# ishine/minimax-speech

Hardware: AMD Instinct MI355X
Metric: 24 kHz audio-seconds generated per wall-second per node (CosyVoice2-0.5B-shaped LM + flow + DAC-VAE, end to end) (higher is better)
Workload: dtype bf16

## Files before the change

### include/mmx_hip.h

```cpp
#ifndef MMX_HIP_H
#define MMX_HIP_H
#include <stdint.h>
#ifdef __cplusplus
extern "C" {
#endif

#ifndef __HIP__
typedef struct ihipStream_t* hipStream_t;
#endif

#define MMX_F32 0
#define MMX_BF16 1
#define MMX_X2 2
#define MMX_X3 3
#define MMX_X2W 0x12
#define MMX_X3W 0x13
#define MMX_H2 4
#define MMX_H2W 0x14

#define MMX_ACT_NONE 0
#define MMX_ACT_LRELU 1
#define MMX_ACT_GELU 2
#define MMX_ACT_SILU 3
#define MMX_ACT_MISH 4
// ... 70 lines not shown
int mmx_attn_flash_x(const float* q, int64_t ldq, int64_t q_bs, const float* k, int64_t ldk, int64_t k_bs,
                     const float* v, int64_t ldv, int64_t v_bs, float* out, int64_t ldo, int64_t o_bs,
                     int B, int H, int T, float scale, const float* keymask, int64_t km_bs, int chunk,
                     int q_begin, const int32_t* klen, hipStream_t stream);
int mmx_attn_flash_xs(const void* qk, int64_t ldqk, int64_t qk_bs, const void* vt, int64_t ldvt, int64_t vt_bs,
                      float* out, int64_t ldo, int64_t o_bs, int B, int H, int T, float scale, const float* keymask,
                      int64_t km_bs, int chunk, int q_begin, const int32_t* klen, int form, hipStream_t stream);
int mmx_attn_relpos_bf16(const void* q, int64_t ldq, int64_t q_bs, const void* k, int64_t ldk, int64_t k_bs,
                         const void* vt, int64_t ldvt, int64_t vt_bs, const void* pos, int64_t ldp,
                         const float* pos_u, const float* pos_v, void* out, int64_t ldo, int64_t o_bs,
                         int B, int H, int T, float scale, int chunk, const int32_t* klen, hipStream_t stream);

int mmx_attn_flash_fp8(const void* q, int64_t ldq, int64_t q_bs, const void* k, int64_t ldk, int64_t k_bs,
                       const void* vt, int64_t ldvt, int64_t vt_bs, void* out, int64_t ldo, int64_t o_bs,
                       int B, int H, int T, float scale, const float* keymask, int64_t km_bs, int chunk, int q_begin,
                       const int32_t* klen, hipStream_t stream);

int mmx_conv_cin1(const float* x, int64_t x_bs, int T, int C, int k, const float* w, const float* bias, float slope,
                  const float* alpha, float* out_f32, void* out_act, int batch, int dtype, hipStream_t stream);
int mmx_vae_sample(const float* ml, const float* noise, int64_t rows, int D, float* z, float* m, float* logs,
                   hipStream_t stream);
int mmx_mask_rows(void* x, int64_t rows, int C, const float* rowmask, int dtype, hipStream_t stream);
int mmx_pool_rows(const float* x, int64_t x_bs, int rows, int C, int batch, const float* mask, int64_t m_bs, void* out,
                  int64_t ldo, int dtype, hipStream_t stream);
int mmx_prefetch4(const void* p0, int64_t n0, const void* p1, int64_t n1, const void* p2, int64_t n2, const void* p3, int64_t n3,
                  void* sink, int workgroups, hipStream_t stream);
int mmx_resample_linear(const float* x, int64_t rows, int T, int T2, float* out, hipStream_t stream);

int mmx_conv_cout1_tanh(const void* act, int64_t a_bs, int T, int C, int k, const float* w, const float* bias,
                        float slope, int use_tanh, float* out, int64_t o_bs, int batch, int dtype, hipStream_t stream);

#define MMX_X_PACKED 1
#define MMX_OUT_PACKED 2
int mmx_pack_skinny(const void* w, int64_t ldw, int N, int K, const float* kscale, int interleave_half,
                    void* wp, int dtype, hipStream_t stream);
int mmx_skinny_gemm(const void* x, int x_dtype, int64_t ldx, int B, int K, int N, const void* wp,
                    const float* bias, int rs, float eps, int epi, float* out_f32, int64_t ldo_f,
                    void* out_act, int64_t ldo_a, int dtype, int flags, const float* kgamma, hipStream_t stream);

int mmx_decode_prep(const float* x, int64_t ldx, int B, int K, const float* gamma, float* h, int64_t ldh, void* xs,
                    float* ssq, int dtype, hipStream_t stream);
int mmx_skinny2(const void* xs, int B, int K, int N, const void* wp, const float* bias, const float* ssq_in, float eps,
                int epi, float* out, int64_t ldo, void* xs_out, const float* gamma_next, float* ssq_out,
                int tiles_per_wg, int ksplit, float* part, int64_t part_floats, int32_t* tickets, int dtype,
                hipStream_t stream);

int mmx_rope_kv_store(const float* qkv, int64_t ldqkv, int64_t qkv_bs, int B, int rows, int Hq, int Hkv, int D,
                      const float* inv_freq, const int32_t* pos, void* q_out, int64_t ldq, int64_t q_bs,
                      void* kc, void* vc, const int32_t* block_table, int max_pages, int page,
                      int dtype, hipStream_t stream);
int mmx_paged_attn(const void* q, int64_t ldq, int64_t q_bs, int B, int rows, int Hq, int Hkv, int D, float scale,
                   const int32_t* pos, const void* kc, const void* vc, const int32_t* block_table, int max_pages,
                   int page, void* out, int64_t ldo, int64_t o_bs, int dtype, hipStream_t stream);
#define MMX_DA_PACKED 1
#define MMX_DA_PER_HEAD 2
#define MMX_DA_SPLIT 4
#define MMX_DA_H2 8
#define MMX_DA_ONE_HEAD 16
int mmx_decode_attn(const float* qkv, int64_t ldqkv, int B, int Hq, int Hkv, int D, const float* inv_freq,
                    const float* rope_tab, const int32_t* pos, void* kc, void* vc, const int32_t* block_table, int max_pages, int page,
                    float scale, void* out, int64_t ldo, int dtype, int out_packed, hipStream_t stream);
int mmx_decode_attn_fin(const float* qkv, int64_t ldqkv, int B, int Hq, int Hkv, int D, const float* inv_freq,
                        const float* rope_tab, const int32_t* pos, const int32_t* finished, void* kc, void* vc,
                        const int32_t* block_table, int max_pages, int page, float scale, void* out, int64_t ldo, int dtype,
                        int out_packed, hipStream_t stream);
int mmx_swiglu(const float* gu, int64_t ldgu, int rows, int I, void* out, int64_t ldo, int dtype, hipStream_t stream);

int mmx_sample_step(const float* logits, int64_t ldl, int V, int B, int eos_id, int top_k, float top_p,
                    int win_size, float tau_r, uint64_t seed, int32_t* state, int32_t* out_tokens, int max_out,
                    int32_t* sampled, const int32_t* forced, const float* speech_emb, int E, float* next_x,
                    int64_t ldx, float* logp_out, hipStream_t stream);
int mmx_sample_step_tab(const float* logits, int64_t ldl, int V, int B, int eos_id, const int32_t* samp, int32_t* state,
                        int32_t* out_tokens, int max_out, int32_t* sampled, const int32_t* forced, const float* speech_emb,
                        int E, float* next_x, int64_t ldx, float* logp_out, hipStream_t stream);

typedef struct MmxEstNext {
    const void* wqkv;
    const float* n1g;
    const float* n1b;
    void* q_out;
    void* vt_out;
    int64_t q_bs, vt_bs;
    int32_t ldq, ldvt;
} MmxEstNext;
typedef struct MmxEstTailParams {
    const void* ao;
    float* x;
    const void* wo;
    const void* w1;
    const void* w2;
    const float* bo;
    const float* b1;
    const float* b2;
    const float* n3g;
    const float* n3b;
    const float* rowmask;
    void* act_out;
    int64_t ao_bs, x_bs, rm_bs, act_bs;
    int32_t ldao, act_ld, B, T;
    int32_t t_begin;
    float eps;
    MmxEstNext next;
} MmxEstTailParams;
typedef struct MmxEstResnetParams {
    const void* a_in;
    float* x;
// ... 88 lines not shown
```

### minimax-speech_amd/csrc/elementwise.hip

```cpp
#include "common.h"
#include <type_traits>

template <int V> using ic = std::integral_constant<int, V>;

template <typename T, int MAXV, int ACT>
__global__ __launch_bounds__(256) void rownorm_kernel(
    const float* __restrict__ x, long ldx, long x_bs, int rows, int C,
    const float* __restrict__ gamma, const float* __restrict__ beta, float eps, int rms, int act,
    const float* __restrict__ rowmask, long rm_bs, const float* __restrict__ addvec, long av_bs,
    float* __restrict__ outf, long ldo_f, long of_bs, T* __restrict__ outa, long ldo_a, long oa_bs) {
    constexpr bool PRECISE = sizeof(T) == 4;
    const int lane = threadIdx.x & 63, wave = threadIdx.x >> 6;
    const int b = blockIdx.y;
    const int row = blockIdx.x * 4 + wave;
    if (row >= rows) return;
    const float* xr = x + (long)b * x_bs + (long)row * ldx;
    float v[MAXV];
    float s = 0.f;
#pragma unroll
    for (int i = 0; i < MAXV; ++i) {
        int c = lane + i * 64;
        v[i] = c < C ? xr[c] : 0.f;
        s += v[i];
    }
// ... 128 lines not shown
                            void* h, int64_t ldh, int dtype, hipStream_t stream) {
    dtype = MMX_ACT_DTYPE(dtype);
    MMX_CHECK_ARG(x && h && B > 0 && T_ > 0 && C > 0 && ldh >= 4 * C && x_mod > 0);
    dim3 grid(T_, B);
    return dispatch_dtype(dtype, [&](auto el) {
        hipLaunchKernelGGL(est_pack_kernel<decltype(el)>, grid, dim3(128), 0, stream, x, x_bs, x_mod, mu, spks, cond, T_, C, (decltype(el)*)h, ldh);
        return launch_status();
    });
}

template <typename T>
__global__ void sinusoidal_kernel(const float* __restrict__ t, int dim, float scale, T* __restrict__ out) {
    const int b = blockIdx.x;
    const int half = dim / 2;
    const float k = logf(10000.f) / (float)(half - 1);
    for (int i = threadIdx.x; i < dim; i += blockDim.x) {
        int j = i < half ? i : i - half;
        float e = scale * t[b] * expf((float)j * -k);
        out[(long)b * dim + i] = Cvt<T>::from_f(i < half ? sinf(e) : cosf(e));
    }
}
extern "C" int mmx_sinusoidal_emb(const float* t, int B, int dim, float scale, void* out, int dtype, hipStream_t stream) {
    dtype = MMX_ACT_DTYPE(dtype);
    MMX_CHECK_ARG(t && out && B > 0 && dim >= 4 && dim % 2 == 0);
    return dispatch_dtype(dtype, [&](auto el) {
        hipLaunchKernelGGL(sinusoidal_kernel<decltype(el)>, dim3(B), dim3(128), 0, stream, t, dim, scale, (decltype(el)*)out);
        return launch_status();
    });
}

__global__ void cfg_euler_kernel(float* __restrict__ x, const float* __restrict__ dc, const float* __restrict__ du,
                                 float cfg, float dt, long n) {
    long i = (long)blockIdx.x * blockDim.x + threadIdx.x;
    if (i < n) x[i] = x[i] + dt * ((1.0f + cfg) * dc[i] - cfg * du[i]);
}
extern "C" int mmx_cfg_euler(float* x, const float* d_cond, const float* d_uncond, float cfg, float dt, int64_t n,
                             hipStream_t stream) {
    MMX_CHECK_ARG(x && d_cond && d_uncond && n > 0);
    hipLaunchKernelGGL(cfg_euler_kernel, dim3((unsigned)((n + 255) / 256)), dim3(256), 0, stream, x, d_cond, d_uncond, cfg, dt, (long)n);
    MMX_LAUNCH_CHECK();
    return MMX_OK;
}

template <typename T>
__global__ __launch_bounds__(256) void conv_cout1_kernel(const T* __restrict__ act, long a_bs, int Tn, int C, int k,
                                                         const float* __restrict__ w, const float* __restrict__ bias,
                                                         float slope, int use_tanh, float* __restrict__ out, long o_bs) {
    extern __shared__ __attribute__((aligned(16))) char smem[];
    float* ws = reinterpret_cast<float*>(smem);
    T* xs = reinterpret_cast<T*>(ws + k * C);
    const int b = blockIdx.y;
    const int t0 = blockIdx.x * 256;
    const int pad = (k - 1) / 2;
    const T* a = act + (long)b * a_bs;
    for (int i = threadIdx.x; i < k * C; i += 256) ws[i] = w[i];
    const int nrow = 256 + k - 1;
    for (int i = threadIdx.x; i < nrow * C; i += 256) {
        int r = i / C, c = i % C;
        long t = (long)t0 + r - pad;
        xs[i] = (t >= 0 && t < Tn) ? a[t * C + c] : Cvt<T>::from_f(0.f);
    }
    __syncthreads();
    const int t = t0 + threadIdx.x;
    if (t >= Tn) return;
    float acc = bias ? bias[0] : 0.f;
    const T* xr = xs + threadIdx.x * C;
    for (int i = 0; i < k * C; ++i) acc += Cvt<T>::to_f(xr[i]) * ws[i];
    acc = acc > 0.f ? acc : acc * slope;
    out[(long)b * o_bs + t] = use_tanh ? tanhf(acc) : fminf(fmaxf(acc, -1.f), 1.f);
}
extern "C" int mmx_conv_cout1_tanh(const void* act, int64_t a_bs, int T_, int C, int k, const float* w, const float* bias,
                                   float slope, int use_tanh, float* out, int64_t o_bs, int batch, int dtype, hipStream_t stream) {
    dtype = MMX_ACT_DTYPE(dtype);
    MMX_CHECK_ARG(act && w && out && T_ > 0 && C > 0 && k > 0 && (k & 1) && batch > 0);
    dim3 grid((T_ + 255) / 256, batch);
    size_t esz = dtype == MMX_BF16 ? 2 : 4;
    size_t lds = (size_t)k * C * 4 + (size_t)(256 + k - 1) * C * esz;
    MMX_CHECK_ARG(lds <= 160 * 1024);
    return dispatch_dtype(dtype, [&](auto el) {
        MMX_LDS_OPT_IN(conv_cout1_kernel<decltype(el)>, lds);
        hipLaunchKernelGGL(conv_cout1_kernel<decltype(el)>, grid, dim3(256), lds, stream, (const decltype(el)*)act, a_bs, T_, C, k, w, bias, slope, use_tanh, out, o_bs);
        return launch_status();
    });
}

template <typename T>
__global__ __launch_bounds__(256) void conv_cin1_kernel(const float* __restrict__ x, long x_bs, int Tn, int C, int k,
                                                        const float* __restrict__ w, const float* __restrict__ bias, float slope,
                                                        const float* __restrict__ alpha, float* __restrict__ outf, T* __restrict__ outa) {
    constexpr bool PRECISE = sizeof(T) == 4;
    extern __shared__ __attribute__((aligned(16))) char smem[];
    float* xs = reinterpret_cast<float*>(smem);
    float* ws = xs + (256 + k - 1);
    const int b = blockIdx.y, t0 = blockIdx.x * 256, pad = (k - 1) / 2;
    const float* xb = x + (long)b * x_bs;
    for (int i = threadIdx.x; i < 256 + k - 1; i += 256) {
        long t = (long)t0 + i - pad;
        xs[i] = (t >= 0 && t < Tn) ? xb[t] : 0.f;
    }
    for (int i = threadIdx.x; i < C * k; i += 256) ws[i] = w[i];
    __syncthreads();
    const int cg = C / 8;
    for (int item = threadIdx.x; item < 256 * cg; item += 256) {
        const int ts = item / cg, c0 = (item % cg) * 8;
        const int t = t0 + ts;
        if (t >= Tn) continue;
        float v[8];
#pragma unroll
        for (int e = 0; e < 8; ++e) {
            float a = bias ? bias[c0 + e] : 0.f;
            for (int j = 0; j < k; ++j) a += ws[(c0 + e) * k + j] * xs[ts + j];
            a = a > 0.f ? a : a * slope;
            v[e] = a;
        }
        const long o = ((long)b * Tn + t) * C + c0;
        if (outf) {
#pragma unroll
            for (int e = 0; e < 8; ++e) outf[o + e] = v[e];
        }
        if (outa) {
#pragma unroll
            for (int e = 0; e < 8; ++e) outa[o + e] = Cvt<T>::from_f(alpha ? snake_apply<PRECISE>(v[e], alpha[c0 + e]) : v[e]);
        }
    }
}
extern "C" int mmx_conv_cin1(const float* x, int64_t x_bs, int T_, int C, int k, const float* w, const float* bias, float slope,
                             const float* alpha, float* out_f32, void* out_act, int batch, int dtype, hipStream_t stream) {
    dtype = MMX_ACT_DTYPE(dtype);
    MMX_CHECK_ARG(x && w && (out_f32 || out_act) && T_ > 0 && C > 0 && C % 8 == 0 && k > 0 && (k & 1) && batch > 0);
    dim3 grid((T_ + 255) / 256, batch);
// ... 221 lines not shown
```

### minimax-speech_amd/csrc/llm.hip

```cpp
#include "act_layout.h"
#include <type_traits>

template <typename T>
__global__ void pack_skinny_kernel(const T* __restrict__ w, long ldw, int N, int K, const float* __restrict__ kscale,
                                   int half, T* __restrict__ wp) {
    constexpr int E = sizeof(T) == 2 ? 8 : 4;
    constexpr int KB = E * 4;
    const long total = (long)((N + 15) / 16) * (K / KB) * 64 * E;
    for (long idx = (long)blockIdx.x * blockDim.x + threadIdx.x; idx < total; idx += (long)gridDim.x * blockDim.x) {
        int j = idx % E;
        long t = idx / E;
        int lane = t % 64;
        t /= 64;
        int kb = t % (K / KB);
        int tile = t / (K / KB);
        int col = lane & 15, g = lane >> 4;
        int row;
        if (half > 0) row = (tile & 1) * half + (tile >> 1) * 16 + col;
        else row = tile * 16 + col;
        int kk = kb * KB + g * E + j;
        float v = 0.f;
        if (row < N && (half == 0 || ((tile >> 1) * 16 + col) < half)) {
            v = Cvt<T>::to_f(w[(long)row * ldw + kk]);
            if (kscale) v *= kscale[kk];
// ... 380 lines not shown
    const int ctx = pos[b] + t + 1;
    const int32_t* bt = block_table + (long)b * max_pages;
    if (tid < D) qs[tid] = Cvt<T>::to_f(q[(long)b * q_bs + (long)t * ldq + h * D + tid]);
    __syncthreads();
    float mx = -INFINITY;
    for (int j = tid; j < ctx; j += 256) {
        const T* kp = kc + (((long)bt[j / page] * Hkv + hk) * page + j % page) * D;
        float s = 0.f;
#pragma unroll
        for (int d = 0; d < D; ++d) s += qs[d] * Cvt<T>::to_f(kp[d]);
        s *= scale;
        S[j] = s;
        mx = fmaxf(mx, s);
    }
    mx = wave_max(mx);
    if (lane == 0) red[wave] = mx;
    __syncthreads();
    mx = fmaxf(fmaxf(red[0], red[1]), fmaxf(red[2], red[3]));
    float l = 0.f;
    for (int j = tid; j < ctx; j += 256) {
        float e = expf(S[j] - mx);
        S[j] = e;
        l += e;
    }
    l = wave_sum(l);
    if (lane == 0) red[4 + wave] = l;
    __syncthreads();
    l = red[4] + red[5] + red[6] + red[7];
    float acc = 0.f;
    for (int j = wave; j < ctx; j += 4) {
        const T* vp = vc + (((long)bt[j / page] * Hkv + hk) * page + j % page) * D;
        acc += S[j] * Cvt<T>::to_f(vp[lane]);
    }
    red[8 + wave * D + lane] = acc;
    __syncthreads();
    if (wave == 0) {
        float o = (red[8 + lane] + red[8 + D + lane]) + (red[8 + 2 * D + lane] + red[8 + 3 * D + lane]);
        out[(long)b * o_bs + (long)t * ldo + h * D + lane] = Cvt<T>::from_f(o / l);
    }
}
extern "C" int mmx_paged_attn(const void* q, int64_t ldq, int64_t q_bs, int B, int rows, int Hq, int Hkv, int D, float scale,
                              const int32_t* pos, const void* kc, const void* vc, const int32_t* block_table, int max_pages,
                              int page, void* out, int64_t ldo, int64_t o_bs, int dtype, hipStream_t stream) {
    dtype = MMX_ACT_DTYPE(dtype);
    MMX_CHECK_ARG(q && pos && kc && vc && block_table && out && B > 0 && rows > 0 && D == 64 && Hq % Hkv == 0 && page > 0);
    const size_t max_ctx = (size_t)max_pages * page;
    size_t lds = (64 + 8 + 4 * 64 + max_ctx) * 4;
    MMX_CHECK_ARG(lds <= 160 * 1024);
    return dispatch_dtype(dtype, [&](auto el) {
        using T = decltype(el);
        MMX_LDS_OPT_IN(paged_attn_kernel<T>, lds);
        hipLaunchKernelGGL(paged_attn_kernel<T>, dim3(Hq, rows, B), dim3(256), lds, stream, (const T*)q, ldq, q_bs, Hq, Hkv, scale, pos, (const T*)kc,
                           (const T*)vc, block_table, max_pages, page, (T*)out, ldo, o_bs);
        return launch_status();
    });
}

template <typename T>
struct Raw8 {
    uint4 a, b;
    __device__ __forceinline__ void load(const T* p) {
        a = *reinterpret_cast<const uint4*>(p);
        if constexpr (sizeof(T) == 4) b = *reinterpret_cast<const uint4*>(p + 4);
    }
    __device__ __forceinline__ void to_float(float o[8]) const {
        const unsigned w[4] = {a.x, a.y, a.z, a.w};
        if constexpr (sizeof(T) == 2) {
#pragma unroll
            for (int i = 0; i < 4; ++i) {
                o[2 * i] = __uint_as_float(w[i] << 16);
                o[2 * i + 1] = __uint_as_float(w[i] & 0xffff0000u);
            }
        } else {
            const unsigned w2[4] = {b.x, b.y, b.z, b.w};
#pragma unroll
            for (int i = 0; i < 4; ++i) { o[i] = __uint_as_float(w[i]); o[4 + i] = __uint_as_float(w2[i]); }
        }
    }
};

constexpr size_t decode_attn_lds(int hp, int max_pages) { return ((size_t)hp * 64 + 2 * 64 + 2 * hp * 32 + (size_t)hp * 32 * 64 + (size_t)max_pages) * 4; }
template <typename T, int OM, int HP>
__global__ __launch_bounds__(256) void decode_attn_kernel(
    const float* __restrict__ qkv, long ldqkv, int Hq, int Hkv, const float* __restrict__ inv_freq,
    const float* __restrict__ rope_tab, const int32_t* __restrict__ pos, T* __restrict__ kc, T* __restrict__ vc,
    const int32_t* __restrict__ block_table, int max_pages, int page, float scale, T* __restrict__ out, long ldo,
    int nseq, const int32_t* __restrict__ finished) {
    constexpr int D = 64, HALF = 32, NG = 32;
    extern __shared__ __attribute__((aligned(16))) char smem[];
    float* qs = reinterpret_cast<float*>(smem);
    float* kn = qs + HP * D;
    float* vn = kn + D;
    float* gm = vn + D;
    float* gl = gm + HP * NG;
    float* part = gl + HP * NG;
    int* bts = reinterpret_cast<int*>(part + HP * NG * D);
    const int tid = threadIdx.x;
    const int group = Hq / Hkv, nsub = (group + HP - 1) / HP;
    const int xcd = blockIdx.x & 7, slot = blockIdx.x >> 3;
    const int kvg = (slot / nsub) * 8 + xcd;
    if (kvg >= Hkv * nseq) return;
    const int b = kvg / Hkv, hk = kvg % Hkv, sub = slot % nsub;
    const int h0 = hk * group + sub * HP, nh = min(HP, group - sub * HP);
    const int p = pos[b];
    if (finished && finished[b]) return;
    const int32_t* bt = block_table + (long)b * max_pages;
// ... 381 lines not shown
```

### minimax-speech_amd/mmx/_lib.py

```python
import ctypes as C
import os

import torch

F32, BF16 = 0, 1
X2, X3 = 2, 3
X2W, X3W = 0x12, 0x13
H2, H2W = 4, 0x14
DA_PACKED, DA_PER_HEAD, DA_SPLIT, DA_H2, DA_ONE_HEAD = 1, 2, 4, 8, 16
ACT = {"none": 0, "lrelu": 1, "gelu": 2, "silu": 3, "mish": 4, "tanh": 5}
TORCH_DT = {F32: torch.float32, BF16: torch.bfloat16, X2: torch.float32, X3: torch.float32, X2W: torch.float32, X3W: torch.float32}
WEIGHT_DT = {F32: torch.float32, BF16: torch.bfloat16, X2: torch.bfloat16, X3: torch.bfloat16, X2W: torch.bfloat16, X3W: torch.bfloat16}
ESIZE = {F32: 4, BF16: 2, X2: 4, X3: 4}
WPLANES = {X2W: 2, X3W: 3}
DTYPE_NAMES = {"f32": F32, "bf16": BF16, "x": X2, "x2": X2, "x3": X3}


def is_split(dtype):
    return dtype in (X2, X3, X2W, X3W)

_HERE = os.path.dirname(os.path.abspath(__file__))
LIB_PATH = os.environ.get("MMX_LIB") or os.path.join(os.path.dirname(_HERE), "lib", "libmmx_hip.so")

SYMBOLS = [
    "mmx_abi_version", "mmx_gemm_win", "mmx_gemm_win_tile", "mmx_rownorm", "mmx_groupnorm", "mmx_act_rows", "mmx_gather_rows", "mmx_copy2d", "mmx_est_pack",
    "mmx_sinusoidal_emb", "mmx_cfg_euler", "mmx_attn_dense", "mmx_attn_flash_bf16", "mmx_attn_flash_fp8", "mmx_attn_relpos_bf16", "mmx_attn_relpos_x", "mmx_attn_flash_x", "mmx_attn_flash_xs", "mmx_conv_cout1_tanh", "mmx_conv_cin1", "mmx_vae_sample", "mmx_resample_linear", "mmx_prefetch4", "mmx_mask_rows",
    "mmx_est_tail", "mmx_est_resnet", "mmx_dac_ru", "mmx_pack_skinny", "mmx_skinny_gemm", "mmx_skinny2", "mmx_decode_prep", "mmx_rope_kv_store", "mmx_paged_attn", "mmx_decode_attn", "mmx_decode_attn_fin", "mmx_swiglu", "mmx_sample_step",
    "mmx_sample_step_tab", "mmx_logmel", "mmx_pool_rows", "mmx_logmel_w", "mmx_s3_rope_fsmn", "mmx_fsq_encode", "mmx_resample_sinc", "mmx_kweight_blocks", "mmx_loudness_gate", "mmx_scale_rows",
    "mmx_spec_dist", "mmx_wave_sums", "mmx_gate_threshold", "mmx_gate_analyze", "mmx_gate_synthesize",
]


class GemmParams(C.Structure):
    _fields_ = [
        ("A", C.c_void_p), ("W", C.c_void_p), ("bias", C.c_void_p), ("residual", C.c_void_p),
        ("rowmask", C.c_void_p), ("alpha", C.c_void_p), ("out_f32", C.c_void_p), ("out_act", C.c_void_p),
        ("lda", C.c_int64), ("ldw", C.c_int64), ("ldr", C.c_int64), ("ldo_f", C.c_int64), ("ldo_a", C.c_int64),
        ("a_bstride", C.c_int64), ("w_bstride", C.c_int64), ("r_bstride", C.c_int64), ("rm_bstride", C.c_int64),
        ("of_bstride", C.c_int64), ("oa_bstride", C.c_int64),
        ("row_off", C.c_int64), ("row_lo", C.c_int64), ("row_hi", C.c_int64),
        ("out_off", C.c_int64), ("out_len", C.c_int64),
        ("M", C.c_int32), ("N", C.c_int32), ("batch", C.c_int32),
        ("ntaps", C.c_int32), ("cin", C.c_int32), ("dil", C.c_int32),
        ("bias_mod", C.c_int32), ("alpha_mod", C.c_int32), ("bias_per_row", C.c_int32),
        ("act", C.c_int32), ("act2", C.c_int32), ("slope", C.c_float), ("row_stride", C.c_int32),
    ]


class EstNext(C.Structure):
    _fields_ = [("wqkv", C.c_void_p), ("n1g", C.c_void_p), ("n1b", C.c_void_p), ("q_out", C.c_void_p), ("vt_out", C.c_void_p),
                ("q_bs", C.c_int64), ("vt_bs", C.c_int64), ("ldq", C.c_int32), ("ldvt", C.c_int32)]


class EstTailParams(C.Structure):
    _fields_ = [(k, C.c_void_p) for k in ("ao", "x", "wo", "w1", "w2", "bo", "b1", "b2", "n3g", "n3b", "rowmask", "act_out")] + \
               [(k, C.c_int64) for k in ("ao_bs", "x_bs", "rm_bs", "act_bs")] + \
               [(k, C.c_int32) for k in ("ldao", "act_ld", "B", "T", "t_begin")] + [("eps", C.c_float), ("next", EstNext)]


class EstResnetParams(C.Structure):
    _fields_ = [(k, C.c_void_p) for k in ("a_in", "x", "w1", "w2", "wr", "b1", "g1", "be1", "b2", "g2", "be2", "br", "tv", "rowmask")] + \
               [(k, C.c_int64) for k in ("a_bs", "x_bs", "tv_bs", "rm_bs")] + \
               [(k, C.c_int32) for k in ("lda", "cin", "B", "T", "t_begin")] + [("eps", C.c_float), ("next", EstNext)]


class DacRuParams(C.Structure):
    _fields_ = [(k, C.c_void_p) for k in ("x", "x_out", "act_out", "w7", "w1", "b7", "b1", "a0", "a2", "alpha_next", "lens")] + \
               [("x_bs", C.c_int64)] + [(k, C.c_int32) for k in ("B", "T", "C", "dil")] + [("slope", C.c_float)]


def fill_struct(st, **kw):
    for k, v in kw.items():
        if v is not None and hasattr(v, "data_ptr"):
            assert v.is_cuda
            v = v.data_ptr()
        setattr(st, k, v)
    return st


ABI_VERSION = 10
# ... 76 lines not shown
```

### minimax-speech_amd/mmx/llm.py

```python
import math
from typing import Dict, List, Optional

import torch

from . import ops
from ._lib import BF16, F32, H2, TORCH_DT, WEIGHT_DT, X3, X3W, is_split
from .flow import Graphed

ST_POS, ST_STEP, ST_NOUT, ST_FIN, ST_MINLEN, ST_MAXLEN, ST_SEQ, ST_ERR = range(8)


class PageAllocator:

    def __init__(self, n_pages: int):
        self.free_pages = list(range(n_pages - 1, -1, -1))
        self.n_pages = n_pages

    @property
    def n_free(self) -> int:
        return len(self.free_pages)

    def alloc(self, n: int) -> List[int]:
        if n > len(self.free_pages):
            raise RuntimeError(f"KV cache exhausted: {n} pages wanted, {len(self.free_pages)} free of {self.n_pages}")
# ... 117 lines not shown
        self.reserve_ahead = 1 << 30

    @staticmethod
    def _dispatch(dtype, h2, wplanes, v2, B, decode_on, prompt_on, gemm_packs):
        planes_only = h2 or wplanes
        packs = ("fp16" if h2 else "bf16") + (" weight-plane" if wplanes else "") + " decode packs"
        decode = "planes" if v2 and dtype != F32 and B <= 32 else "skinny"
        if decode_on not in (None, decode):
            raise ValueError(f"decode_on={decode_on!r}: 'planes' (csrc/decode.hip) serves the bf16 and split builds up to 32 sequences, "
                             f"'skinny' (mmx_skinny_gemm) the rest; this is dtype {dtype} at max_batch {B}")
        if planes_only and decode != "planes":
            raise ValueError(f"{packs} are read by csrc/decode.hip only, which does not serve " +
                             (f"max_batch {B} > 32" if v2 else "the round-2 kernel (use_v2 = False / decode_on='skinny')"))
        ok = ("gemm",) if planes_only else ("gemm", "gemm-batch", "skinny") if gemm_packs else ("skinny",)
        if prompt_on not in (None,) + ok:
            raise ValueError(f"prompt_on={prompt_on!r}: {packs}" + ("" if gemm_packs else ", shared model without row-major copies,") + f" take {ok}")
        return decode, prompt_on or ("gemm" if planes_only else "gemm-batch" if B >= 4 and gemm_packs else "skinny")

    @staticmethod
    def _attn_kw(split, h2, B, gqa_min_batch):
        return dict(per_head=bool(split or B < gqa_min_batch), out_split=("f16" if h2 else bool(split)), out_packed=not split)

    def _layers(self, h, ha, B, rows, pos, block_table, packed=False):
        m = self.model
        dt, H, I = m.dtype, m.H, m.I
        n = B * rows
        assert n <= 64 and not (packed and rows != 1)
        nr = ops.packed_rows(n) if packed else n
        qkv = torch.empty(n, (m.Hq + 2 * m.Hkv) * m.D, device=self.dev)
        q = torch.empty(n, m.Hq * m.D, dtype=m.tdt, device=self.dev)
        att = torch.empty(nr, m.Hq * m.D, dtype=m.tdt, device=self.dev)
        act = torch.empty(nr, I, dtype=m.tdt, device=self.dev)
        kg = (lambda g: g) if m.unfolded else (lambda g: None)
        res = dict(out_f32=h) if m.split else dict(out_f32=h, out_act=ha)
        gu = dict(out_f32=act) if m.split else dict(out_act=act)
        for l, w in enumerate(m.layers):
            first = (packed and l == 0) or m.unfolded
            ops.skinny_gemm(h if first else ha, w["wqkv"], B=n, K=H, N=qkv.shape[1], dtype=dt, bias=w["bqkv"], rs=True,
                            eps=m.eps, epi=0, out_f32=qkv, x_packed=packed and not first, kgamma=kg(w["g1"]))
            if rows == 1:
                ops.decode_attn(qkv, m.inv_freq, pos, m.kc[l], m.vc[l], block_table, att, B=B, Hq=m.Hq,
                                Hkv=m.Hkv, page=m.page, dtype=dt, rope_tab=m.rope_tab, out_packed=packed,
                                per_head=m.split or B < self.gqa_min_batch)
            else:
                ops.rope_kv_store(qkv, m.inv_freq, pos, q, m.kc[l], m.vc[l], block_table, B=B, rows=rows,
                                  Hq=m.Hq, Hkv=m.Hkv, page=m.page, dtype=dt)
                ops.paged_attn(q, pos, m.kc[l], m.vc[l], block_table, att, B=B, rows=rows, Hq=m.Hq,
                               Hkv=m.Hkv, page=m.page, dtype=dt)
            ops.skinny_gemm(att, w["wo"], B=n, K=m.Hq * m.D, N=H, dtype=dt, epi=2, x_packed=packed, out_packed=packed, **res)
            ops.skinny_gemm(h if m.unfolded else ha, w["wgu"], B=n, K=H, N=I, dtype=dt, rs=True, eps=m.eps, epi=1,
                            x_packed=packed, out_packed=packed, kgamma=kg(w["g2"]), **gu)
            ops.skinny_gemm(act, w["wdown"], B=n, K=I, N=H, dtype=dt, epi=2, x_packed=packed, out_packed=packed, **res)

    v2_cfg = dict(qkv=(1, 1), o=(1, 1), gu=(2, 1), down=(2, 8), head=(2, 1))

    def _planes(self):
        if not hasattr(self, "_v2"):
            m = self.model
            H, I, R = m.H, m.I, ops.packed_rows(self.B)
            NQ = (m.Hq + 2 * m.Hkv) * m.D
            bf = lambda K: torch.zeros((2 if m.h2 else 3) if m.split else 1, R * K, dtype=torch.bfloat16, device=self.dev)
            J = self.v2_cfg["down"][1]
            self._v2 = dict(qkv=torch.empty(self.B, NQ, device=self.dev), xs_a=bf(H), xs_b=bf(H), xs_att=bf(m.Hq * m.D), xs_act=bf(I),
                            ssq_a=torch.zeros(32, ops.SSQ_SLOTS, device=self.dev), ssq_b=torch.zeros(32, ops.SSQ_SLOTS, device=self.dev),
                            part=torch.empty(J * ((H + 15) // 16) * (R // 4) * 64, device=self.dev),
                            tickets=torch.zeros((H + 15) // 16, dtype=torch.int32, device=self.dev))
        return self._v2

    def _prefetch(self, l=None):
        if not int(self.prefetch):
            return
        if not hasattr(self, "_pf_side"):
            self._pf_side = torch.cuda.Stream(device=self.dev)
            self._pf_sink = torch.zeros(4, dtype=torch.int32, device=self.dev)
        layers, ev = self.model.layers, torch.cuda.Event()
        src, dst = (torch.cuda.current_stream(), self._pf_side) if l is not None else (self._pf_side, torch.cuda.current_stream())
        ev.record(src)
        dst.wait_event(ev)
        if l is not None:
            with torch.cuda.stream(self._pf_side):
                ops.prefetch4([layers[l + 1][k] for k in ("wqkv", "wo", "wgu", "wdown")] if l + 1 < len(layers) else [self.model.wdec],
                              self._pf_sink, int(self.prefetch))

    def _layers_split_decode(self, x_in, h, B, pos, block_table):
        m = self.model
        dt, H, I, c, S = m.ddt, m.H, m.I, self.v2_cfg, self._planes()
        NQ = (m.Hq + 2 * m.Hkv) * m.D
        qkv = S["qkv"][:B]
        fin = self.state[ST_FIN] if self.skip_finished else None
        ops.decode_prep(x_in, S["xs_a"], S["ssq_a"], B=B, K=H, gamma=m.layers[0]["g1"], h=h, dtype=dt)
        for l, w in enumerate(m.layers):
            self._prefetch(l)
            g_next = m.layers[l + 1]["g1"] if l + 1 < len(m.layers) else m.norm_w
            ops.skinny2(S["xs_a"], w["wqkv"], B=B, K=H, N=NQ, dtype=dt, bias=w["bqkv"], ssq_in=S["ssq_a"], eps=m.eps, epi=0, out=qkv,
                        tiles_per_wg=c["qkv"][0])
            ops.decode_attn(qkv, m.inv_freq, pos, m.kc[l], m.vc[l], block_table, S["xs_att"], B=B, Hq=m.Hq,
                            Hkv=m.Hkv, page=m.page, dtype=m.dtype, rope_tab=m.rope_tab, finished=fin,
                            **self._attn_kw(m.split, m.h2, B, self.gqa_min_batch))
            ops.skinny2(S["xs_att"], w["wo"], B=B, K=m.Hq * m.D, N=H, dtype=dt, epi=2, out=h, xs_out=S["xs_b"],
                        gamma_next=w["g2"], ssq_out=S["ssq_b"], tiles_per_wg=c["o"][0])
            ops.skinny2(S["xs_b"], w["wgu"], B=B, K=H, N=I, dtype=dt, ssq_in=S["ssq_b"], eps=m.eps, epi=1, xs_out=S["xs_act"],
                        tiles_per_wg=c["gu"][0])
            ops.skinny2(S["xs_act"], w["wdown"], B=B, K=I, N=H, dtype=dt, epi=2, out=h, xs_out=S["xs_a"], gamma_next=g_next,
                        ssq_out=S["ssq_a"], tiles_per_wg=c["down"][0], ksplit=c["down"][1], part=S["part"], tickets=S["tickets"])
        self._prefetch(None)

# ... 106 lines not shown
            raise RuntimeError("sequence exceeds the KV cache")
        self.release(slot)
        self._set_pages(slot, L + (max_len if ahead is None else min(ahead, max_len)))
        x = x.to(self.dev, torch.float32).contiguous()
        self._prefill(x[:L - 1], 0, slot)
        self.x_in[slot].copy_(x[L - 1])
        st = torch.tensor([L - 1, 0, 0, 0, min_len, max_len, seq_id, 0], dtype=torch.int32)
        self.state[:, slot].copy_(st)
        self._write_sampler(slot, fields, col)
        self.sampled[slot].fill_(-1)

    def start(self, lm_inputs: List[torch.Tensor], min_lens: List[int], max_lens: List[int], seed=0, seq_ids=None,
              forced: Optional[torch.Tensor] = None, want_logp=False, samplers: Optional[list] = None,
              seeds: Optional[list] = None):
        B = self.B
        assert len(lm_inputs) == B and (samplers is None or len(samplers) == B) and (seeds is None or len(seeds) == B)
        self.seed, self.want_logp = int(seed), want_logp
        self._write_samplers([self._sampler_fields(samplers[b] if samplers else None, seeds[b] if seeds else None) for b in range(B)])
        if forced is not None:
            if self._forced_buf is None:
                self._forced_buf = torch.zeros(B, self.max_out, dtype=torch.int32, device=self.dev)
            self._forced_buf[:, :forced.shape[1]].copy_(forced.to(torch.int32))
            self.forced = self._forced_buf
        else:
            self.forced = None
        st = torch.zeros(8, B, dtype=torch.int32)
        for b in range(B):
            st[ST_MINLEN, b], st[ST_MAXLEN, b] = min_lens[b], max_lens[b]
            st[ST_SEQ, b] = b if seq_ids is None else seq_ids[b]
        self.state.copy_(st)
        self.sampled.fill_(-1)
        for b, x in enumerate(lm_inputs):
            assert x.shape[0] + max_lens[b] <= self.max_pages * self.page, "sequence exceeds the KV cache"
            self.release(b)
            self._set_pages(b, x.shape[0] + min(max_lens[b], self.reserve_ahead))
        if self.prompt_on != "skinny":
            self._prefill_batch(lm_inputs)
        else:
            for b, x in enumerate(lm_inputs):
                self._prefill(x, 0, b, head=True)
                self.state[ST_POS, b] = x.shape[0] - 1
        self._tail(B)
        self._fresh_decode_graph()

    def _prefill_batch(self, lm_inputs):
        B, H = self.B, self.H
        Ls = [int(x.shape[0]) for x in lm_inputs]
        Lm = max(Ls)
        R = B * Lm
        h = torch.zeros(B, Lm, H, device=self.dev)
        for b, x in enumerate(lm_inputs):
            h[b, :Ls[b]].copy_(x)
        h = h.reshape(R, H)
        self._gemm_layers(h, B, Lm, torch.zeros(B, dtype=torch.int32, device=self.dev), self.block_table)
        last = torch.tensor([b * Lm + Ls[b] - 1 for b in range(B)], dtype=torch.long, device=self.dev)
        hl = h.index_select(0, last)
        self.h[:B].copy_(hl)
        self.h_act[:B].copy_(hl)
        self.state[ST_POS].copy_(torch.tensor([L - 1 for L in Ls], dtype=torch.int32))

    def _gemm_layers(self, h, B, Lm, pos, block_table):
        m = self.model
        dt, H, I = m.dtype, m.H, m.I
        R = B * Lm
        a = torch.empty(R, H, dtype=m.tdt, device=self.dev)
        qkv = torch.empty(R, (m.Hq + 2 * m.Hkv) * m.D, device=self.dev)
        q = torch.empty(R, m.Hq * m.D, dtype=m.tdt, device=self.dev)
        att = torch.empty(R, m.Hq * m.D, dtype=m.tdt, device=self.dev)
        gu = torch.empty(R, 2 * I, device=self.dev)
        act = torch.empty(R, I, dtype=m.tdt, device=self.dev)
        for l, (w, ws) in enumerate(zip(m.pf_layers, m.layers)):
            ops.rownorm(h, w["g1"], None, m.eps, rows=R, C_=H, rms=True, out_act=a, dtype=dt)
            ops.linear(a, w["wqkv"], H, dtype=dt, bias=ws["bqkv"], out_f32=qkv)
            ops.rope_kv_store(qkv, m.inv_freq, pos, q, m.kc[l], m.vc[l], block_table, B=B, rows=Lm,
                              Hq=m.Hq, Hkv=m.Hkv, page=m.page, dtype=dt)
            ops.paged_attn(q, pos, m.kc[l], m.vc[l], block_table, att, B=B, rows=Lm, Hq=m.Hq,
                           Hkv=m.Hkv, page=m.page, dtype=dt)
            ops.linear(att, w["wo"], m.Hq * m.D, dtype=dt, residual=h, out_f32=h)
            ops.rownorm(h, w["g2"], None, m.eps, rows=R, C_=H, rms=True, out_act=a, dtype=dt)
            ops.linear(a, w["wgu"], H, dtype=dt, out_f32=gu)
            ops.swiglu(gu, act, rows=R, I=I, dtype=dt)
            ops.linear(act, w["wdown"], I, dtype=dt, residual=h, out_f32=h)

    def _prefill(self, x, pos0, slot, head=False, norm_out=None):
        m = self.model
        x = x.to(self.dev, torch.float32).contiguous()
        for c0 in range(0, x.shape[0], 64):
            hc, hca = self._prefill_chunk(x[c0:c0 + 64], pos0 + c0, slot)
            if norm_out is not None:
                ops.rownorm(hc, m.norm_w, None, m.eps, rows=hc.shape[0], C_=m.H, rms=True, out_f32=norm_out[c0:c0 + 64], dtype=F32)
        if head:
            self.h[slot].copy_(hc[-1])
            self.h_act[slot].copy_(hca[-1])

    def _prefill_chunk(self, xc, pos0, b):
        rows = xc.shape[0]
        if self.prompt_on == "gemm":
            hc = xc.to(self.dev, torch.float32).clone()
            self._gemm_layers(hc, 1, rows, torch.tensor([pos0], dtype=torch.int32, device=self.dev), self.block_table[b:b + 1].contiguous())
            return hc, hc.to(self.tdt)
        if not hasattr(self, "_pf"):
            self._pf = dict(h=torch.zeros(64, self.H, device=self.dev), ha=torch.zeros(64, self.H, dtype=self.tdt, device=self.dev),
                            pos=torch.zeros(1, dtype=torch.int32, device=self.dev),
                            bt=torch.zeros(1, self.max_pages, dtype=torch.int32, device=self.dev), graphs={})
        pf = self._pf
        pf["h"][:rows].copy_(xc)
        pf["ha"][:rows].copy_(xc)
        pf["pos"].fill_(pos0)
        pf["bt"].copy_(self.block_table[b:b + 1])
        if rows not in pf["graphs"]:
            pf["graphs"][rows] = Graphed(lambda r=rows: self._layers(pf["h"][:r], pf["ha"][:r], 1, r, pf["pos"], pf["bt"]), self.use_graphs)
        pf["graphs"][rows]()
        return pf["h"][:rows], pf["ha"][:rows]

    def step(self):
        self._decode()

    def close(self):
        if self._decode is not None:
            self._decode.release()
            self._decode = None
        if hasattr(self, "_pf"):
            for g in self._pf["graphs"].values():
                g.release()
            del self._pf

    @torch.no_grad()
    def forward_rows(self, x: torch.Tensor, pos0: int) -> torch.Tensor:
        n = x.shape[0]
        if pos0 + n > self.max_pages * self.page:
            raise RuntimeError("sequence exceeds the KV cache")
        if pos0 == 0:
            self.release(0)
        self._set_pages(0, pos0 + n)
        out = torch.empty(n, self.H, device=self.dev)
        self._prefill(x, pos0, 0, norm_out=out)
        return out

    def compact_from(self, big: "LlmEngine", idx: List[int]):
        n = len(idx)
        assert n <= self.B and big.kc is self.kc
        ii = torch.tensor(idx, dtype=torch.long, device=self.dev)
        st = torch.zeros(8, self.B, dtype=torch.int32, device=self.dev)
        st[ST_FIN, n:] = 1
        st[:, :n] = big.state[:, ii]
        self.state.copy_(st)
        self.out_tokens[:n].copy_(big.out_tokens[ii])
        self.sampled[:n].copy_(big.sampled[ii])
        self.x_in[:n].copy_(big.x_in[ii])
        self.block_table.fill_(self.model.trash_page)
        self.block_table[:n].copy_(big.block_table[ii])
        self.seed, self.want_logp = big.seed, False
# ... 145 lines not shown
```

### minimax-speech_amd/mmx/ops.py

```python
import ctypes as C
import math

import torch

from . import _lib as L
from ._lib import ACT, BF16, F32, check, i64, load, stream, _p


def round_up(x, m):
    return (x + m - 1) // m * m


class Planed(torch.Tensor):
    """A packed weight held as bf16 PLANES hi + [mid +] lo = w of an fp32 checkpoint's values (include/mmx_hip.h MMX_X2W / MMX_X3W).
    The type is the marker: gemm() / skinny2() switch to the weight-plane dtype code when they are handed one; views and row
    slices keep the type (torch's default __torch_function__)."""


def weight_planes(w: torch.Tensor, n: int):
    out, r = [], w.float()
    for _ in range(n):
        t = r.to(torch.bfloat16)
        out.append(t)
        r = r - t.float()
# ... 358 lines not shown


def merge_planes(xs, B, K, f16=False):
    if f16:
        return sum(unpack_act(xs[s], B, K, BF16).contiguous().view(torch.float16).float() for s in range(2))
    return sum(unpack_act(xs[s], B, K, BF16).float() for s in range(3))


H2_WSCALE = 256.0


def pack_skinny_h2(w, *, planes=1, interleave_half=0):
    ws = w.float() * H2_WSCALE
    assert float(ws.abs().max()) < 65504.0, "weight out of the fp16 range of MMX_H2"
    out, r = [], ws
    for _ in range(planes):
        t = r.to(torch.float16)
        out.append(pack_skinny(t.view(torch.bfloat16).contiguous(), dtype=L.X3, interleave_half=interleave_half))
        r = r - t.float()
    return out[0] if planes == 1 else torch.cat(out).as_subclass(Planed)


def decode_prep(x, xs, ssq, *, B, K, gamma=None, h=None, dtype=L.X3):
    check(load().mmx_decode_prep(_p(x), i64(x.shape[-1]), B, K, _p(gamma), _p(h), i64(h.shape[-1] if h is not None else 0), _p(xs),
                                 _p(ssq), dtype, stream()), "mmx_decode_prep")


def skinny2(xs, wp, *, B, K, N, dtype, bias=None, ssq_in=None, eps=1e-6, epi=0, out=None, ldo=None, xs_out=None, gamma_next=None,
            ssq_out=None, tiles_per_wg=1, ksplit=1, part=None, tickets=None):
    if isinstance(wp, Planed):
        dtype = L.H2W if dtype in (L.H2, L.H2W) else L.X3W
    check(load().mmx_skinny2(_p(xs), B, K, N, _p(wp), _p(bias), _p(ssq_in), C.c_float(eps), epi, _p(out),
                             i64(ldo if ldo is not None else N), _p(xs_out), _p(gamma_next), _p(ssq_out), tiles_per_wg, ksplit,
                             _p(part), i64(part.numel() if part is not None else 0), _p(tickets), dtype, stream()), "mmx_skinny2")


def rope_kv_store(qkv, inv_freq, pos, q_out, kc, vc, block_table, *, B, rows, Hq, Hkv, page, dtype, ldqkv=None, qkv_bs=None,
                  ldq=None, q_bs=None):
    ldqkv = (Hq + 2 * Hkv) * 64 if ldqkv is None else ldqkv
    ldq = Hq * 64 if ldq is None else ldq
    check(load().mmx_rope_kv_store(_p(qkv), i64(ldqkv), i64(rows * ldqkv if qkv_bs is None else qkv_bs), B, rows, Hq, Hkv, 64,
                                   _p(inv_freq), _p(pos), _p(q_out), i64(ldq), i64(rows * ldq if q_bs is None else q_bs), _p(kc), _p(vc),
                                   _p(block_table), block_table.shape[1], page, dtype, stream()), "mmx_rope_kv_store")


def paged_attn(q, pos, kc, vc, block_table, out, *, B, rows, Hq, Hkv, page, dtype, ldq=None, q_bs=None, ldo=None, o_bs=None):
    ldq = Hq * 64 if ldq is None else ldq
    ldo = Hq * 64 if ldo is None else ldo
    check(load().mmx_paged_attn(_p(q), i64(ldq), i64(rows * ldq if q_bs is None else q_bs), B, rows, Hq, Hkv, 64, C.c_float(0.125),
                                _p(pos), _p(kc), _p(vc), _p(block_table), block_table.shape[1], page, _p(out),
                                i64(ldo), i64(rows * ldo if o_bs is None else o_bs), dtype, stream()), "mmx_paged_attn")


def decode_attn_bits(out_packed=False, per_head=False, out_split=False, one_head=False):
    return ((L.DA_PACKED if out_packed else 0) | (L.DA_PER_HEAD if per_head else 0) | (L.DA_ONE_HEAD if one_head else 0) |
            (L.DA_H2 if out_split == "f16" else L.DA_SPLIT if out_split else 0))


def decode_attn(qkv, inv_freq, pos, kc, vc, block_table, out, *, B, Hq, Hkv, page, dtype, rope_tab=None, out_packed=False,
                per_head=False, out_split=False, one_head=False, ldqkv=None, ldo=None, finished=None):
    assert finished is None or (finished.dtype == torch.int32 and finished.numel() >= B and finished.stride(-1) == 1)
    check(load().mmx_decode_attn_fin(_p(qkv), i64((Hq + 2 * Hkv) * 64 if ldqkv is None else ldqkv), B, Hq, Hkv, 64, _p(inv_freq), _p(rope_tab),
                                     _p(pos), _p(finished), _p(kc), _p(vc), _p(block_table), block_table.shape[1], page, C.c_float(0.125), _p(out),
                                     i64(Hq * 64 if ldo is None else ldo), dtype, decode_attn_bits(out_packed, per_head, out_split, one_head), stream()), "mmx_decode_attn_fin")


def swiglu(gu, out, *, rows, I, dtype, ldgu=None, ldo=None):
    check(load().mmx_swiglu(_p(gu), i64(ldgu or 2 * I), rows, I, _p(out), i64(ldo or I), dtype, stream()), "mmx_swiglu")


def sample_step(logits, state, out_tokens, speech_emb, next_x, *, V, B, eos_id, seed, top_k=25, top_p=0.8,
                win_size=10, tau_r=0.1, sampled=None, forced=None, logp_out=None):
    check(load().mmx_sample_step(_p(logits), i64(logits.shape[-1]), V, B, eos_id, top_k, C.c_float(top_p), win_size,
                                 C.c_float(tau_r), C.c_uint64(seed), _p(state), _p(out_tokens), out_tokens.shape[1],
                                 _p(sampled), _p(forced), _p(speech_emb), speech_emb.shape[1], _p(next_x),
                                 i64(next_x.shape[-1]), _p(logp_out), stream()), "mmx_sample_step")


SAMP_MODE, SAMP_TOP_K, SAMP_WIN, SAMP_TOP_P, SAMP_TAU_R, SAMP_SEED_LO, SAMP_SEED_HI = range(7)
SAMPLER_MODES = {"ras": 0, "nucleus": 1, "random": 2}


def sampler_column(mode=0, top_p=0.8, top_k=25, win_size=10, tau_r=0.1, seed=0):
    import struct
    mode = SAMPLER_MODES.get(mode, mode)
    if mode not in (0, 1, 2) or not 1 <= int(top_k) <= 64 or not 0 <= int(win_size) <= 64:
        raise ValueError(f"sampler out of range: mode {mode!r} (0..2), top_k {top_k} (1..64), win_size {win_size} (0..64)")
    bits = lambda v: struct.unpack("<i", struct.pack("<f", float(v)))[0]
    i32 = lambda u: u - (1 << 32) if u >= (1 << 31) else u
    seed = int(seed) & ((1 << 64) - 1)
    return [int(mode), int(top_k), int(win_size), bits(top_p), bits(tau_r), i32(seed & 0xffffffff), i32(seed >> 32), 0]


def sample_step_tab(logits, state, out_tokens, speech_emb, next_x, samp, *, V, B, eos_id, sampled=None, forced=None, logp_out=None):
    assert samp.dtype == torch.int32 and samp.is_contiguous() and samp.shape == (8, B)
    check(load().mmx_sample_step_tab(_p(logits), i64(logits.shape[-1]), V, B, eos_id, _p(samp), _p(state), _p(out_tokens),
                                     out_tokens.shape[1], _p(sampled), _p(forced), _p(speech_emb), speech_emb.shape[1],
                                     _p(next_x), i64(next_x.shape[-1]), _p(logp_out), stream()), "mmx_sample_step_tab")
```

Measured before the change: 571.1.

## Add LDS-tiled prompt attention kernel sharing KV across query rows and GQA heads

Adds a prompt-prefill attention kernel that stages a whole KV-head's keys and values into LDS once per block of four query rows, then has each wave run the softmax attention for every query head in that KV group. This replaces the per-(head,row) paged_attn kernel, which reread the KV cache repeatedly. It falls back to paged_attn when the context exceeds the LDS capacity. Separately, the cout1 conv kernel pads its LDS rows (C+1) to avoid bank conflicts and drops the per-element divide/modulo in the staging loop. The cost is much higher LDS use per block, which may limit occupancy.

```diff
diff --git a/include/mmx_hip.h b/include/mmx_hip.h
--- a/include/mmx_hip.h
+++ b/include/mmx_hip.h
@@ -146,6 +146,10 @@
 int mmx_paged_attn(const void* q, int64_t ldq, int64_t q_bs, int B, int rows, int Hq, int Hkv, int D, float scale,
                    const int32_t* pos, const void* kc, const void* vc, const int32_t* block_table, int max_pages,
                    int page, void* out, int64_t ldo, int64_t o_bs, int dtype, hipStream_t stream);
+#define MMX_PROMPT_ATTN_LDS_PER_KEY 536
+int mmx_prompt_attn(const void* q, int64_t ldq, int64_t q_bs, int B, int rows, int Hq, int Hkv, int D, float scale,
+                    const int32_t* pos, const void* kc, const void* vc, const int32_t* block_table, int max_pages,
+                    int page, int nk_max, void* out, int64_t ldo, int64_t o_bs, int dtype, hipStream_t stream);
 #define MMX_DA_PACKED 1
 #define MMX_DA_PER_HEAD 2
 #define MMX_DA_SPLIT 4
diff --git a/minimax-speech_amd/csrc/elementwise.hip b/minimax-speech_amd/csrc/elementwise.hip
--- a/minimax-speech_amd/csrc/elementwise.hip
+++ b/minimax-speech_amd/csrc/elementwise.hip
@@ -204,20 +204,24 @@
     const int b = blockIdx.y;
     const int t0 = blockIdx.x * 256;
     const int pad = (k - 1) / 2;
+    const int ld = C + 1;
     const T* a = act + (long)b * a_bs;
     for (int i = threadIdx.x; i < k * C; i += 256) ws[i] = w[i];
     const int nrow = 256 + k - 1;
-    for (int i = threadIdx.x; i < nrow * C; i += 256) {
-        int r = i / C, c = i % C;
-        long t = (long)t0 + r - pad;
-        xs[i] = (t >= 0 && t < Tn) ? a[t * C + c] : Cvt<T>::from_f(0.f);
+    const int dr = 256 / C, dc = 256 % C;
+    for (int r = (int)threadIdx.x / C, c = (int)threadIdx.x % C; r < nrow; r += dr) {
+        const long t = (long)t0 + r - pad;
+        xs[r * ld + c] = (t >= 0 && t < Tn) ? a[t * C + c] : Cvt<T>::from_f(0.f);
+        c += dc;
+        if (c >= C) c -= C, ++r;
     }
     __syncthreads();
     const int t = t0 + threadIdx.x;
     if (t >= Tn) return;
     float acc = bias ? bias[0] : 0.f;
-    const T* xr = xs + threadIdx.x * C;
-    for (int i = 0; i < k * C; ++i) acc += Cvt<T>::to_f(xr[i]) * ws[i];
+    const T* xr = xs + threadIdx.x * ld;
+    for (int j = 0; j < k; ++j)
+        for (int c = 0; c < C; ++c) acc += Cvt<T>::to_f(xr[j * ld + c]) * ws[j * C + c];
     acc = acc > 0.f ? acc : acc * slope;
     out[(long)b * o_bs + t] = use_tanh ? tanhf(acc) : fminf(fmaxf(acc, -1.f), 1.f);
 }
@@ -227,7 +231,7 @@
     MMX_CHECK_ARG(act && w && out && T_ > 0 && C > 0 && k > 0 && (k & 1) && batch > 0);
     dim3 grid((T_ + 255) / 256, batch);
     size_t esz = dtype == MMX_BF16 ? 2 : 4;
-    size_t lds = (size_t)k * C * 4 + (size_t)(256 + k - 1) * C * esz;
+    size_t lds = (size_t)k * C * 4 + (size_t)(256 + k - 1) * (C + 1) * esz;
     MMX_CHECK_ARG(lds <= 160 * 1024);
     return dispatch_dtype(dtype, [&](auto el) {
         MMX_LDS_OPT_IN(conv_cout1_kernel<decltype(el)>, lds);
diff --git a/minimax-speech_amd/csrc/llm.hip b/minimax-speech_amd/csrc/llm.hip
--- a/minimax-speech_amd/csrc/llm.hip
+++ b/minimax-speech_amd/csrc/llm.hip
@@ -456,6 +456,124 @@
         MMX_LDS_OPT_IN(paged_attn_kernel<T>, lds);
         hipLaunchKernelGGL(paged_attn_kernel<T>, dim3(Hq, rows, B), dim3(256), lds, stream, (const T*)q, ldq, q_bs, Hq, Hkv, scale, pos, (const T*)kc,
                            (const T*)vc, block_table, max_pages, page, (T*)out, ldo, o_bs);
+        return launch_status();
+    });
+}
+
+constexpr int PA_ROWS = 4, PA_LD = 65;
+template <typename T>
+__device__ __forceinline__ void load4f(const T* p, float o[4]) {
+    if constexpr (sizeof(T) == 4) {
+        const float4 v = *reinterpret_cast<const float4*>(p);
+        o[0] = v.x, o[1] = v.y, o[2] = v.z, o[3] = v.w;
+    } else {
+        const uint2 v = *reinterpret_cast<const uint2*>(p);
+        o[0] = __uint_as_float(v.x << 16), o[1] = __uint_as_float(v.x & 0xffff0000u);
+        o[2] = __uint_as_float(v.y << 16), o[3] = __uint_as_float(v.y & 0xffff0000u);
+    }
+}
+template <typename T>
+__global__ __launch_bounds__(64 * PA_ROWS) void prompt_attn_kernel(
+    const T* __restrict__ q, long ldq, long q_bs, int rows, int Hq, int Hkv, float scale, const int32_t* __restrict__ pos,
+    const T* __restrict__ kc, const T* __restrict__ vc, const int32_t* __restrict__ block_table, int max_pages,
+    int page, int nk_max, T* __restrict__ out, long ldo, long o_bs) {
+    constexpr int D = 64;
+    extern __shared__ __attribute__((aligned(16))) char smem[];
+    float* Ks = reinterpret_cast<float*>(smem);
+    float* Vs = Ks + (long)nk_max * PA_LD;
+    float* Sw = Vs + (long)nk_max * PA_LD;
+    const int tid = threadIdx.x, lane = tid & 63, wave = __builtin_amdgcn_readfirstlane(tid >> 6);
+    const int r0 = blockIdx.x * PA_ROWS, hk = blockIdx.y, b = blockIdx.z;
+    const int G = Hq / Hkv;
+    const int p0 = pos[b];
+    const int nr = min(PA_ROWS, rows - r0);
+    const int nk = p0 + r0 + nr;
+    const int t = r0 + wave;
+    if (p0 < 0 || nk > nk_max) {
+        if (wave < nr)
+            for (int g = 0; g < G; ++g) out[(long)b * o_bs + (long)t * ldo + (hk * G + g) * D + lane] = Cvt<T>::from_f(NAN);
+        return;
+    }
+    const int32_t* bt = block_table + (long)b * max_pages;
+    int* krow = reinterpret_cast<int*>(Sw);
+    for (int j = tid; j < nk; j += 64 * PA_ROWS) krow[j] = (bt[j / page] * Hkv + hk) * page + j % page;
+    __syncthreads();
+#pragma unroll 4
+    for (int i = tid; i < nk * (D / 4); i += 64 * PA_ROWS) {
+        const int j = i >> 4, d0 = (i & 15) * 4;
+        const long row = (long)krow[j] * D + d0;
+        float kf[4], vf[4];
+        load4f(kc + row, kf);
+        load4f(vc + row, vf);
+#pragma unroll
+        for (int e = 0; e < 4; ++e) {
+            Ks[j * PA_LD + d0 + e] = kf[e];
+            Vs[j * PA_LD + d0 + e] = vf[e];
+        }
+    }
+    __syncthreads();
+    if (wave >= nr) return;
+    const int ctx = p0 + t + 1;
+    float* S = Sw + (long)wave * nk_max;
+    for (int g = 0; g < G; ++g) {
+        const int h = hk * G + g;
+        const float qv = Cvt<T>::to_f(q[(long)b * q_bs + (long)t * ldq + h * D + lane]);
+        float mx = -INFINITY;
+        for (int j0 = 0; j0 < ctx; j0 += 64) {
+            const int j = j0 + lane;
+            const float* kp = Ks + min(j, ctx - 1) * PA_LD;
+            float s = 0.f;
+#pragma unroll
+            for (int d = 0; d < D; ++d) s += __int_as_float(__builtin_amdgcn_readlane(__float_as_int(qv), d)) * kp[d];
+            s *= scale;
+            if (j < ctx) {
+                S[j] = s;
+                mx = fmaxf(mx, s);
+            }
+        }
+        mx = wave_max(mx);
+        float lp[4] = {0.f, 0.f, 0.f, 0.f};
+        for (int j0 = 0; j0 < ctx; j0 += 256) {
+#pragma unroll
+            for (int w = 0; w < 4; ++w) {
+                const int j = j0 + w * 64 + lane;
+                if (j < ctx) {
+                    float e = expf(S[j] - mx);
+                    S[j] = e;
+                    lp[w] += e;
+                }
+            }
+        }
+        const float l = wave_sum(lp[0]) + wave_sum(lp[1]) + wave_sum(lp[2]) + wave_sum(lp[3]);
+        __builtin_amdgcn_wave_barrier();
+        float acc[4] = {0.f, 0.f, 0.f, 0.f};
+        const float* vp = Vs + lane;
+        int j = 0;
+        for (; j + 4 <= ctx; j += 4) {
+#pragma unroll
+            for (int w = 0; w < 4; ++w) acc[w] += S[j + w] * vp[(j + w) * PA_LD];
+        }
+        for (int w = 0; j + w < ctx; ++w) acc[w] += S[j + w] * vp[(j + w) * PA_LD];
+        const float o = (acc[0] + acc[1]) + (acc[2] + acc[3]);
+        out[(long)b * o_bs + (long)t * ldo + h * D + lane] = Cvt<T>::from_f(o / l);
+        __builtin_amdgcn_wave_barrier();
+    }
+}
+static_assert(MMX_PROMPT_ATTN_LDS_PER_KEY == (2 * PA_LD + PA_ROWS) * 4, "include/mmx_hip.h states the kernel's LDS per key row");
+extern "C" int mmx_prompt_attn(const void* q, int64_t ldq, int64_t q_bs, int B, int rows, int Hq, int Hkv, int D, float scale,
+                               const int32_t* pos, const void* kc, const void* vc, const int32_t* block_table, int max_pages,
+                               int page, int nk_max, void* out, int64_t ldo, int64_t o_bs, int dtype, hipStream_t stream) {
+    dtype = MMX_ACT_DTYPE(dtype);
+    MMX_CHECK_ARG(q && pos && kc && vc && block_table && out && B > 0 && rows > 0 && D == 64 && Hkv > 0 && Hq % Hkv == 0 && page > 0);
+    MMX_CHECK_ARG(nk_max >= rows && (size_t)nk_max <= (size_t)max_pages * page);
+    const size_t lds = (size_t)nk_max * MMX_PROMPT_ATTN_LDS_PER_KEY;
+    MMX_CHECK_ARG(lds <= 160 * 1024);
+    return dispatch_dtype(dtype, [&](auto el) {
+        using T = decltype(el);
+        MMX_LDS_OPT_IN(prompt_attn_kernel<T>, lds);
+        hipLaunchKernelGGL(prompt_attn_kernel<T>, dim3((rows + PA_ROWS - 1) / PA_ROWS, Hkv, B), dim3(64 * PA_ROWS), lds, stream, (const T*)q,
+                           ldq, q_bs, rows, Hq, Hkv, scale, pos, (const T*)kc, (const T*)vc, block_table, max_pages, page, nk_max, (T*)out,
+                           ldo, o_bs);
         return launch_status();
     });
 }
diff --git a/minimax-speech_amd/mmx/_lib.py b/minimax-speech_amd/mmx/_lib.py
--- a/minimax-speech_amd/mmx/_lib.py
+++ b/minimax-speech_amd/mmx/_lib.py
@@ -25,7 +25,7 @@
 SYMBOLS = [
     "mmx_abi_version", "mmx_gemm_win", "mmx_gemm_win_tile", "mmx_rownorm", "mmx_groupnorm", "mmx_act_rows", "mmx_gather_rows", "mmx_copy2d", "mmx_est_pack",
     "mmx_sinusoidal_emb", "mmx_cfg_euler", "mmx_attn_dense", "mmx_attn_flash_bf16", "mmx_attn_flash_fp8", "mmx_attn_relpos_bf16", "mmx_attn_relpos_x", "mmx_attn_flash_x", "mmx_attn_flash_xs", "mmx_conv_cout1_tanh", "mmx_conv_cin1", "mmx_vae_sample", "mmx_resample_linear", "mmx_prefetch4", "mmx_mask_rows",
-    "mmx_est_tail", "mmx_est_resnet", "mmx_dac_ru", "mmx_pack_skinny", "mmx_skinny_gemm", "mmx_skinny2", "mmx_decode_prep", "mmx_rope_kv_store", "mmx_paged_attn", "mmx_decode_attn", "mmx_decode_attn_fin", "mmx_swiglu", "mmx_sample_step",
+    "mmx_est_tail", "mmx_est_resnet", "mmx_dac_ru", "mmx_pack_skinny", "mmx_skinny_gemm", "mmx_skinny2", "mmx_decode_prep", "mmx_rope_kv_store", "mmx_paged_attn", "mmx_prompt_attn", "mmx_decode_attn", "mmx_decode_attn_fin", "mmx_swiglu", "mmx_sample_step",
     "mmx_sample_step_tab", "mmx_logmel", "mmx_pool_rows", "mmx_logmel_w", "mmx_s3_rope_fsmn", "mmx_fsq_encode", "mmx_resample_sinc", "mmx_kweight_blocks", "mmx_loudness_gate", "mmx_scale_rows",
     "mmx_spec_dist", "mmx_wave_sums", "mmx_gate_threshold", "mmx_gate_analyze", "mmx_gate_synthesize",
 ]
diff --git a/minimax-speech_amd/mmx/llm.py b/minimax-speech_amd/mmx/llm.py
--- a/minimax-speech_amd/mmx/llm.py
+++ b/minimax-speech_amd/mmx/llm.py
@@ -193,6 +193,8 @@
                             x_packed=packed, out_packed=packed, kgamma=kg(w["g2"]), **gu)
             ops.skinny_gemm(act, w["wdown"], B=n, K=I, N=H, dtype=dt, epi=2, x_packed=packed, out_packed=packed, **res)
 
+    prompt_attn_tiled = True
+
     v2_cfg = dict(qkv=(1, 1), o=(1, 1), gu=(2, 1), down=(2, 8), head=(2, 1))
 
     def _planes(self):
@@ -405,14 +407,14 @@
         for b, x in enumerate(lm_inputs):
             h[b, :Ls[b]].copy_(x)
         h = h.reshape(R, H)
-        self._gemm_layers(h, B, Lm, torch.zeros(B, dtype=torch.int32, device=self.dev), self.block_table)
+        self._gemm_layers(h, B, Lm, torch.zeros(B, dtype=torch.int32, device=self.dev), self.block_table, Lm)
         last = torch.tensor([b * Lm + Ls[b] - 1 for b in range(B)], dtype=torch.long, device=self.dev)
         hl = h.index_select(0, last)
         self.h[:B].copy_(hl)
         self.h_act[:B].copy_(hl)
         self.state[ST_POS].copy_(torch.tensor([L - 1 for L in Ls], dtype=torch.int32))
 
-    def _gemm_layers(self, h, B, Lm, pos, block_table):
+    def _gemm_layers(self, h, B, Lm, pos, block_table, max_ctx):
         m = self.model
         dt, H, I = m.dtype, m.H, m.I
         R = B * Lm
@@ -427,8 +429,8 @@
             ops.linear(a, w["wqkv"], H, dtype=dt, bias=ws["bqkv"], out_f32=qkv)
             ops.rope_kv_store(qkv, m.inv_freq, pos, q, m.kc[l], m.vc[l], block_table, B=B, rows=Lm,
                               Hq=m.Hq, Hkv=m.Hkv, page=m.page, dtype=dt)
-            ops.paged_attn(q, pos, m.kc[l], m.vc[l], block_table, att, B=B, rows=Lm, Hq=m.Hq,
-                           Hkv=m.Hkv, page=m.page, dtype=dt)
+            ops.prompt_attn(q, pos, m.kc[l], m.vc[l], block_table, att, B=B, rows=Lm, Hq=m.Hq,
+                            Hkv=m.Hkv, page=m.page, dtype=dt, max_ctx=max_ctx, tiled=self.prompt_attn_tiled)
             ops.linear(att, w["wo"], m.Hq * m.D, dtype=dt, residual=h, out_f32=h)
             ops.rownorm(h, w["g2"], None, m.eps, rows=R, C_=H, rms=True, out_act=a, dtype=dt)
             ops.linear(a, w["wgu"], H, dtype=dt, out_f32=gu)
@@ -450,7 +452,8 @@
         rows = xc.shape[0]
         if self.prompt_on == "gemm":
             hc = xc.to(self.dev, torch.float32).clone()
-            self._gemm_layers(hc, 1, rows, torch.tensor([pos0], dtype=torch.int32, device=self.dev), self.block_table[b:b + 1].contiguous())
+            self._gemm_layers(hc, 1, rows, torch.tensor([pos0], dtype=torch.int32, device=self.dev), self.block_table[b:b + 1].contiguous(),
+                              pos0 + rows)
             return hc, hc.to(self.tdt)
         if not hasattr(self, "_pf"):
             self._pf = dict(h=torch.zeros(64, self.H, device=self.dev), ha=torch.zeros(64, self.H, dtype=self.tdt, device=self.dev),
diff --git a/minimax-speech_amd/mmx/ops.py b/minimax-speech_amd/mmx/ops.py
--- a/minimax-speech_amd/mmx/ops.py
+++ b/minimax-speech_amd/mmx/ops.py
@@ -434,6 +434,21 @@
                                 i64(ldo), i64(rows * ldo if o_bs is None else o_bs), dtype, stream()), "mmx_paged_attn")
 
 
+PROMPT_ATTN_MAX_KEYS = 160 * 1024 // 536
+
+
+def prompt_attn(q, pos, kc, vc, block_table, out, *, B, rows, Hq, Hkv, page, dtype, max_ctx, tiled=True, **pitch):
+    if not tiled or max_ctx > PROMPT_ATTN_MAX_KEYS:
+        paged_attn(q, pos, kc, vc, block_table, out, B=B, rows=rows, Hq=Hq, Hkv=Hkv, page=page, dtype=dtype, **pitch)
+        return "paged"
+    ldq, ldo = (Hq * 64 if pitch.get(k) is None else pitch[k] for k in ("ldq", "ldo"))
+    q_bs, o_bs = (rows * ld if pitch.get(k) is None else pitch[k] for k, ld in (("q_bs", ldq), ("o_bs", ldo)))
+    check(load().mmx_prompt_attn(_p(q), i64(ldq), i64(q_bs), B, rows, Hq, Hkv, 64, C.c_float(0.125), _p(pos), _p(kc), _p(vc),
+                                 _p(block_table), block_table.shape[1], page, int(max_ctx), _p(out), i64(ldo), i64(o_bs), dtype, stream()),
+          "mmx_prompt_attn")
+    return "tiled"
+
+
 def decode_attn_bits(out_packed=False, per_head=False, out_split=False, one_head=False):
     return ((L.DA_PACKED if out_packed else 0) | (L.DA_PER_HEAD if per_head else 0) | (L.DA_ONE_HEAD if one_head else 0) |
             (L.DA_H2 if out_split == "f16" else L.DA_SPLIT if out_split else 0))
```

Result: no change. 573.6 (median of 6 runs) (+0.4%).
